# lusinlu/Video-Generation-for-Human-Avatars

Hardware: AMD Instinct MI355X
Metric: LTX-2B LoRA train-step samples/sec (latent-tokens/sec = samples/sec x 1792) (higher is better)
Workload: dtype bf16; 1 GPU; LTX-Video 2B LoRA(r=16, attn2 q/k/v/out) + caption_projection train step, 49f 512x512 -> latent 7x16x16 (N=1792), 1xMI355X per rank; lora_rank=16, model=LTX-Video-2B (28 layers, D 2048, 32x64 heads), global_batch=8, micro_batch_per_gpu=8, seq_len=1792, text_len=256, grad_accum=16, parallelism=dp1, attn2_padding_blocks=skipped, exact

## Files before the change

include/ltx_hip.h:

```cpp
#ifndef LTX_HIP_H_
#define LTX_HIP_H_

#include <stdint.h>

#ifdef __cplusplus
extern "C" {
#endif

enum {
  LTX_OK = 0,
  LTX_ERR_BAD_ARG = 1000,
  LTX_ERR_UNSUPPORTED = 1001,
};

enum {
  LTX_EPI_STORE = 0,
  LTX_EPI_GELU = 1,
  LTX_EPI_GATED_RESIDUAL = 2,
  LTX_EPI_LORA = 3,
  LTX_EPI_LORA_RESIDUAL = 4,
  LTX_EPI_GELU_BWD = 5,
  LTX_EPI_ACCUM = 6,
  LTX_EPI_LORA_DGRAD_ACCUM = 7,
  LTX_EPI_STORE_ROWDOT = 8,
// ... 132 lines not shown
                    int64_t ldo, void* stream);
int ltx_lora_rows(const void* x, int64_t ldx, const void* w3, int64_t ldw, float* out, int64_t ldo,
                  int64_t M, int64_t K, int64_t r, float alpha, void* split, int64_t ld_split,
                  int64_t K2, void* stream);
int ltx_lora_wgrad(const void* y, int64_t ldy, const float* u, int64_t ldu, float* dw,
                   int64_t on, int64_t oj, int64_t M, int64_t N, int64_t r, float alpha,
                   int accumulate, void* stream);
int ltx_lora_wgrad_grouped(const void* y, int64_t ldy, const float* u, int64_t ldu, float* dw,
                           int64_t on, int64_t oj, int64_t M, int64_t N, int64_t r, float alpha,
                           int accumulate, int64_t groups, int64_t gy, int64_t gu, int64_t gd,
                           void* stream);

int ltx_lora_dy(const void* y, int64_t ldy, const float* u, int64_t ldu, const void* w3, int64_t ldw3,
                int64_t M, int64_t N, int64_t r, float alpha, float* w, int64_t ldw_out, void* split,
                int64_t ld_split, int64_t K2, float* dw, int64_t on, int64_t oj, int accumulate,
                float* workspace, void* stream);
int ltx_lora_dy_workspace(int64_t M, int64_t N, int64_t r, int64_t* floats);
int ltx_lora_dy_dA(const void* y, int64_t ldy, const float* u, int64_t ldu, const void* w3, int64_t ldw3,
                   const void* x, int64_t ldx, int64_t M, int64_t N, int64_t K, int64_t r, float alpha,
                   float* w, int64_t ldw_out, void* split, int64_t ld_split, int64_t K2, float* dw,
                   int64_t on, int64_t oj, int accumulate, float alpha_a, float* dwa, int64_t ona,
                   int64_t oja, int acc_a, float* workspace, void* stream);
int ltx_lora_dy_dA_workspace(int64_t M, int64_t N, int64_t K, int64_t r, int64_t* floats);
int ltx_lora_rows_grouped(const void* x, int64_t ldx, const void* const* w3, int64_t ldw, float* out,
                          int64_t ldo, int64_t go, int64_t M, int64_t K, int64_t r, float alpha,
                          void* split, int64_t ld_split, int64_t K2, int64_t gs, int64_t groups,
                          void* stream);
int ltx_lora_dy_dA_grouped(const void* y, int64_t ldy, const float* const* u, int64_t ldu,
                           const void* const* w3, int64_t ldw3, const void* x, int64_t ldx, int64_t M,
                           int64_t N, int64_t K, int64_t r, int64_t groups, float alpha, float* w,
                           int64_t ldw_out, int64_t gw, void* split, int64_t ld_split, int64_t K2,
                           int64_t gs, float* const* dw, int64_t on, int64_t oj, int accumulate,
                           float alpha_a, float* const* dwa, int64_t ona, int64_t oja, int acc_a,
                           float* workspace, void* stream);
int ltx_lora_dy_dA_grouped_workspace(int64_t M, int64_t N, int64_t K, int64_t r, int64_t groups,
                                     int64_t* floats);

int ltx_lora_dropout_apply(const void* x, int64_t ldx, void* out, int64_t ldo, int64_t M, int64_t K,
                           uint64_t key, int64_t sid, int64_t T, void* stream);
int ltx_lora_up_masked_add(void* dx, int64_t lddx, const float* w, int64_t ldw, const float* const* A,
                           int64_t lda, const int64_t* sids, int64_t groups, int64_t M, int64_t K,
                           int64_t r, uint64_t key, int64_t T, float c, const void* gq, int64_t ldg,
                           void* stream);

int ltx_dora_fold(const void* W, int64_t ldw, const float* A, int64_t lda, const float* B, int64_t brs,
                  int64_t bcs, const float* m, float s, int64_t N, int64_t K, int64_t r, float* norm,
// ... 62 lines not shown
```

video-generation-for-human-avatars_amd/csrc/lora_dy.hip:

```cpp
#include <cstdlib>

#include "attention_common.h"
#include "ltx_hip.h"

namespace ltx {

#ifndef LTX_RF_NR
#define LTX_RF_NR 5
#endif
namespace {
constexpr int DY_NR = 4;
constexpr int DY_COLS = 512;
constexpr int DY_MAXCS = 4;
constexpr int dy_sw(int r) { return r <= 16 ? 16 : 32; }
constexpr int dy_g(int r) { return r <= 16 ? 7 : 4; }
constexpr int dy_nsl(int r) { return r <= 32 ? 1 : r / 32; }
constexpr bool dy_rank_ok(int64_t r) { return r == 8 || r == 16 || r == 32 || r == 64 || r == 128; }
}

template <int R, int MODE>
__global__ __launch_bounds__(512) void lora_dy_kernel(const bf16_t* __restrict__ y, int64_t ldy,
                                                      const float* __restrict__ u, int64_t ldu,
                                                      const bf16_t* __restrict__ w3, int64_t ldw,
                                                      float* __restrict__ part_w, float* __restrict__ part_b,
                                                      int M, int N, const float* __restrict__ part_u, int CSu,
                                                      float alpha_u) {
#define DY_BX blockIdx.x
#define DY_BY blockIdx.y
#define LTX_DY_BODY 1
#include "lora_dy_bodies.h"
#undef LTX_DY_BODY
#undef DY_BX
#undef DY_BY
}

constexpr int LORA_MAX_GROUPS = 4;
struct DyGroupPtrs {
  const float* u[LORA_MAX_GROUPS];
  const bf16_t* w3[LORA_MAX_GROUPS];
  float* dw[LORA_MAX_GROUPS];
  float* dwa[LORA_MAX_GROUPS];
};

template <int R, int MODE>
__global__ __launch_bounds__(512) void lora_dy_grouped_kernel(const bf16_t* __restrict__ y0, int64_t ldy,
                                                              DyGroupPtrs gp, int64_t ldu, int64_t ldw,
                                                              float* __restrict__ part_w0,
                                                              float* __restrict__ part_b0, int M, int N,
                                                              const float* __restrict__ part_u0, int CSu,
                                                              float alpha_u, int G, int64_t gy, int64_t gpw,
                                                              int64_t gpb, int64_t gpu) {
  unsigned g, gbx;
  if constexpr ((MODE & 4) != 0) {
// ... 61 lines not shown

template <int R>
__global__ __launch_bounds__(256) void lora_dy_finish_grouped_kernel(
    const float* __restrict__ part_w0, int CS, const float* __restrict__ part_b0, int RS, int M, int N, float alpha,
    float* __restrict__ w0, int64_t ldw_out, bf16_t* __restrict__ split0, int64_t lds, int K2, DyGroupPtrs gp,
    int64_t on, int64_t oj, int accumulate, int nwb, int nbb, const float* __restrict__ part_a0, int Na,
    float alpha_a, int64_t ona, int64_t oja, int acc_a, int64_t gpw, int64_t gpb, int64_t gpa, int64_t gwo,
    int64_t gso) {
  const unsigned g = blockIdx.y;
  const float* __restrict__ part_w = part_w0 + g * gpw;
  const float* __restrict__ part_b = part_b0 + g * gpb;
  const float* __restrict__ part_a = part_a0 + g * gpa;
  float* __restrict__ w = w0 + g * gwo;
  bf16_t* __restrict__ split = split0 + g * gso;
  float* __restrict__ dw = gp.dw[g];
  float* __restrict__ dwa = gp.dwa[g];
#define DY_BX blockIdx.x
#define DY_BY blockIdx.y
#define LTX_DY_BODY 2
#include "lora_dy_bodies.h"
#undef LTX_DY_BODY
#undef DY_BX
#undef DY_BY
}

template <int R, int RG, int CH, int NR>
__global__ __launch_bounds__(512) void lora_rows_full_kernel(const bf16_t* __restrict__ x, int64_t ldx,
                                                             const bf16_t* __restrict__ w3, int64_t ldw,
                                                             float* __restrict__ out, int64_t ldo, int M, float alpha,
                                                             bf16_t* __restrict__ split, int64_t lds, int K2) {
#define DY_BX blockIdx.x
#define DY_BY blockIdx.y
#define LTX_DY_BODY 3
#include "lora_dy_bodies.h"
#undef LTX_DY_BODY
#undef DY_BX
#undef DY_BY
}

struct RowsGroupPtrs {
  const bf16_t* w3[LORA_MAX_GROUPS];
};
template <int R, int RG, int CH, int NR>
__global__ __launch_bounds__(512) void lora_rows_full_grouped_kernel(const bf16_t* __restrict__ x, int64_t ldx,
                                                                     RowsGroupPtrs gp, int64_t ldw,
                                                                     float* __restrict__ out0, int64_t ldo, int M,
// ... 202 lines not shown
                     ldy, u, ldu, (const bf16_t*)w3, ldw3, pw, pb, (int)M, (int)N, (const float*)nullptr, 0, 1.f);  \
  LTX_LAUNCH_CHECK();                                                                                              \
  if (CS <= DY_MAXCS)                                                                                              \
    hipLaunchKernelGGL((lora_dy_kernel<RR, 6>), dim3((unsigned)(CSx * NSL), (unsigned)RS), dim3(512), 0, s,       \
                       (const bf16_t*)x, ldx, (const float*)nullptr, (int64_t)0, (const bf16_t*)nullptr,           \
                       (int64_t)0, (float*)nullptr, pa, (int)M, (int)K, (const float*)pw, CS, alpha);              \
  else                                                                                                             \
    hipLaunchKernelGGL((lora_dy_kernel<RR, 14>), dim3((unsigned)(CSx * NSL), (unsigned)RS), dim3(512), 0, s,      \
                       (const bf16_t*)x, ldx, (const float*)nullptr, (int64_t)0, (const bf16_t*)nullptr,           \
                       (int64_t)0, (float*)nullptr, pa, (int)M, (int)K, (const float*)pw, CS, alpha);              \
  LTX_LAUNCH_CHECK();                                                                                              \
  hipLaunchKernelGGL((lora_dy_finish_kernel<RR>), dim3((unsigned)(nwb + nbb + nba)), dim3(256), 0, s, pw, CS, pb,  \
                     RS, (int)M, (int)N, alpha, w, ldw_out, (bf16_t*)split, ld_split, (int)K2, dw, on, oj,         \
                     accumulate, nwb, nbb, (const float*)pa, (int)K, alpha_a, dwa, ona, oja, acc_a);
  switch (r) {
    case 8: LTX_LORA_DYA(8) break;
    case 16: LTX_LORA_DYA(16) break;
    case 32: LTX_LORA_DYA(32) break;
    case 64: LTX_LORA_DYA(64) break;
    case 128: LTX_LORA_DYA(128) break;
    default: return fail(LTX_ERR_BAD_ARG, "lora_dy_dA: rank must be 8, 16, 32, 64 or 128");
  }
#undef LTX_LORA_DYA
  LTX_LAUNCH_CHECK();
  return LTX_OK;
}

extern "C" int ltx_lora_dy_dA_grouped_workspace(int64_t M, int64_t N, int64_t K, int64_t r, int64_t groups,
                                                int64_t* floats) {
  LTX_CHECK_ARG(groups >= 1 && groups <= LORA_MAX_GROUPS, "lora_dy_dA_grouped_workspace: 1 to 4 groups");
  int64_t one = 0;
  const int rc = ltx_lora_dy_dA_workspace(M, N, K, r, &one);
  if (rc != LTX_OK) return rc;
  *floats = groups * one;
  return LTX_OK;
}

extern "C" int ltx_lora_dy_dA_grouped(const void* y, int64_t ldy, const float* const* u, int64_t ldu,
                                      const void* const* w3, int64_t ldw3, const void* x, int64_t ldx, int64_t M,
                                      int64_t N, int64_t K, int64_t r, int64_t groups, float alpha, float* w,
                                      int64_t ldw_out, int64_t gw, void* split, int64_t ld_split, int64_t K2,
                                      int64_t gs, float* const* dw, int64_t on, int64_t oj, int accumulate,
                                      float alpha_a, float* const* dwa, int64_t ona, int64_t oja, int acc_a,
                                      float* workspace, void* stream) {
  LTX_CHECK_ARG(y && u && w3 && x && w && split && dw && dwa && workspace, "lora_dy_dA_grouped: null operand");
  LTX_CHECK_ARG(groups >= 1 && groups <= LORA_MAX_GROUPS, "lora_dy_dA_grouped: 1 to 4 groups");
// ... 130 lines not shown
```

video-generation-for-human-avatars_amd/csrc/lora_dy_bodies.h:

```cpp
#if LTX_DY_BODY == 1
  constexpr int RP = R >= 16 ? R : 16;
  constexpr int SW = dy_sw(R);
  constexpr int NSL = dy_nsl(R);
  constexpr int DY_G = dy_g(R);
  constexpr int DY_UPAD = DY_G * 32 + 4;
  constexpr int JT = SW / 16;
  constexpr int NF = 3 * JT;
  constexpr int RING = 8 * DY_NR * 4096;
  constexpr int UT = SW * DY_UPAD * 4;
  static_assert(dy_rank_ok(R), "rank 8, 16, 32, 64 or 128");
  __shared__ __attribute__((aligned(16))) char smem[RING + UT];
  float* ut = (float*)(smem + RING);
  const int tid = threadIdx.x, lane = tid & 63;
  const int wave = __builtin_amdgcn_readfirstlane(tid >> 6);
  const int cs = DY_BX / NSL, rs = DY_BY;
  const int j0 = (DY_BX % NSL) * SW;
  const int c0 = cs * DY_COLS + wave * 64;
  const int mb = rs * DY_G * 32;

  uint32_t yo[4];
#pragma unroll
  for (int i = 0; i < 4; ++i) {
    const int row = 8 * i + (lane >> 3);
    yo[i] = (uint32_t)(row * ldy + (((lane & 7) ^ swz<64>(row)) * 8)) * 2;
// ... 81 lines not shown
#pragma unroll
      for (int c = 0; c < DY_MAXCS; ++c)
        if (c < CSu) acc += pv[i][c];
      uv[i] = (e < DY_G * 32 * SW && m < M && j < R) ? acc * alpha_u : 0.f;
    }
#pragma unroll
    for (int i = 0; i < UPT; ++i) {
      const int e = tid + 512 * i;
      if (e < DY_G * 32 * SW) ut[(e / (DY_G * 32)) * DY_UPAD + e % (DY_G * 32)] = uv[i];
    }
  } else {
#pragma unroll
    for (int i = 0; i < UPT; ++i) {
      const int e = tid + 512 * i, rr = e / SW, j = j0 + e % SW, m = mb + rr;
      uv[i] = ((MODE & 2) && e < DY_G * 32 * SW && m < M && j < R) ? u[(int64_t)m * ldu + j] : 0.f;
    }
#pragma unroll
    for (int i = 0; i < UPT; ++i) {
      const int e = tid + 512 * i;
      if ((MODE & 2) && e < DY_G * 32 * SW) ut[(e % SW) * DY_UPAD + e / SW] = uv[i];
    }
  }
  __syncthreads();

  int roff[2][2];
#pragma unroll
  for (int q = 0; q < 2; ++q)
#pragma unroll
    for (int h = 0; h < 2; ++h) {
      const int row = 16 * q + (lane & 15);
      roff[q][h] = row * 128 + (((4 * h + (lane >> 4)) ^ swz<64>(row)) * 16);
    }
  const int g4 = lane >> 4, qq = (lane & 15) >> 2, pp = lane & 3;
  int toffs[4];
#pragma unroll
  for (int nb = 0; nb < 4; ++nb) toffs[nb] = toff<64>(4 * g4 + qq, 2 * nb + (pp >> 1)) + 8 * (pp & 1);
  auto tr4 = [](const char* a) {
    return __builtin_amdgcn_ds_read_tr16_b64_v4i16((__attribute__((address_space(3))) s16x4*)a);
  };

  f32x4 wacc[DY_G][2][JT];
  f32x4 bacc[JT][4];
#pragma unroll
  for (int t = 0; t < JT; ++t)
#pragma unroll
    for (int nb = 0; nb < 4; ++nb) bacc[t][nb] = (f32x4){0.f, 0.f, 0.f, 0.f};
// ... 287 lines not shown
```

video-generation-for-human-avatars_amd/ltx_amd/_lib.py:

```python
import ctypes
import os
import threading

import torch

_HERE = os.path.dirname(os.path.abspath(__file__))
LIB_PATH = os.environ.get("LTX_HIP_LIB", os.path.join(_HERE, "libltxhip.so"))

_i64 = ctypes.c_int64
_i32 = ctypes.c_int
_f32 = ctypes.c_float
_p = ctypes.c_void_p

_SIGNATURES = {
    "ltx_abi_version": [],
    "ltx_device_info": [ctypes.POINTER(_i32), ctypes.POINTER(_i32)],
    "ltx_patchify_bf16": [_p, _p, _i64, _i64, _i64, _i64, _i64, _p],
    "ltx_unpatchify_bf16": [_p, _p, _i64, _i64, _i64, _i64, _i64, _p],
    "ltx_latent_coords": [_p, _i64, _i64, _i64, _i64, _p],
    "ltx_rf_noise_velocity": [_p, _p, _p, _p, _p, _i64, _i64, _p],
    "ltx_rf_noise_velocity_f32": [_p, _i32, _p, _i32, _p, _p, _p, _i64, _i64, _p],
    "ltx_condition_lerp": [_p, _p, _p, _p, _i64, _i64, _i64, _i64, _i64, _p],
    "ltx_rf_prepare_tokens": [_p, _p, _p, _p, _p, _p, _p, _p, _i64, _i64, _i64, _i64, _i64, _p],
    "ltx_rmsnorm_modulate_fwd": [_p, _p, _p, _i64, _p, _p, _i64, _i64, _i64, _f32, _p],
# ... 27 lines not shown
    "ltx_gemm_set_variant": [_i32],
    "ltx_gemm_describe": [_i64, _i64, _i64, _i64, _i32, _i64, _p, _p, _i64],
    "ltx_add_bf16": [_p, _i64, _p, _i64, _p, _i64, _i64, _i64, _p],
    "ltx_gated_residual_bf16": [_p, _i64, _p, _i64, _p, _i64, _p, _i64, _i64, _i64, _i64, _p],
    "ltx_gemm_set_workspace": [_p, _i64],
    "ltx_gemm_set_stream_workspace": [_p, _p, _i64],
    "ltx_gemm_bf16_nt_ext": [_p, _i64, _p, _i64, _p, _i64, _p, _i64, _i64, _p, _i64, _i64, _i64,
                             _i64, _i32, _p, _p, _i64, _p, _i64, _p, _i64, _f32, _i64, _i64, _p],
    "ltx_gemm_bf16_nt_gext": [_p, _i64, _p, _i64, _p, _i64, _p, _i64, _i64, _i64, _i64, _p, _i64,
                              _i64, _i64, _i64, _i32, _p, _p, _i64, _p, _i64, _p, _i64, _f32, _i64,
                              _i64, _p],
    "ltx_lora_down_grouped": [_p, _i64, _p, _i64, _i64, _p, _i64, _i64, _i64, _i64, _f32, _p, _i64,
                              _i64, _i64, _i64, _i64, _i64, _i64, _p],
    "ltx_lora_wgrad_grouped": [_p, _i64, _p, _i64, _p, _i64, _i64, _i64, _i64, _i64, _f32, _i32,
                               _i64, _i64, _i64, _i64, _p],
    "ltx_lora_pieces": [_p, _i64, _i64, _i64, _i64, _p, _i64, _p],
    "ltx_lora_rows": [_p, _i64, _p, _i64, _p, _i64, _i64, _i64, _i64, _f32, _p, _i64, _i64, _p],
    "ltx_lora_dy": [_p, _i64, _p, _i64, _p, _i64, _i64, _i64, _i64, _f32, _p, _i64, _p, _i64, _i64, _p,
                    _i64, _i64, _i32, _p, _p],
    "ltx_lora_dy_workspace": [_i64, _i64, _i64, ctypes.POINTER(_i64)],
    "ltx_lora_dy_dA": [_p, _i64, _p, _i64, _p, _i64, _p, _i64, _i64, _i64, _i64, _i64, _f32, _p, _i64,
                       _p, _i64, _i64, _p, _i64, _i64, _i32, _f32, _p, _i64, _i64, _i32, _p, _p],
    "ltx_lora_dy_dA_workspace": [_i64, _i64, _i64, _i64, ctypes.POINTER(_i64)],
    "ltx_lora_rows_grouped": [_p, _i64, ctypes.POINTER(_p), _i64, _p, _i64, _i64, _i64, _i64, _i64, _f32,
                              _p, _i64, _i64, _i64, _i64, _p],
    "ltx_lora_dy_dA_grouped": [_p, _i64, ctypes.POINTER(_p), _i64, ctypes.POINTER(_p), _i64, _p, _i64, _i64,
                               _i64, _i64, _i64, _i64, _f32, _p, _i64, _i64, _p, _i64, _i64, _i64,
                               ctypes.POINTER(_p), _i64, _i64, _i32, _f32, ctypes.POINTER(_p), _i64, _i64,
                               _i32, _p, _p],
    "ltx_lora_dy_dA_grouped_workspace": [_i64, _i64, _i64, _i64, _i64, ctypes.POINTER(_i64)],
    "ltx_lora_dropout_apply": [_p, _i64, _p, _i64, _i64, _i64, ctypes.c_uint64, _i64, _i64, _p],
    "ltx_lora_up_masked_add": [_p, _i64, _p, _i64, ctypes.POINTER(_p), _i64, ctypes.POINTER(_i64), _i64, _i64,
                               _i64, _i64, ctypes.c_uint64, _i64, _f32, _p, _i64, _p],
    "ltx_dora_fold": [_p, _i64, _p, _i64, _p, _i64, _i64, _p, _f32, _i64, _i64, _i64, _p, _p, _p, _i64, _p, _p],
    "ltx_dora_mag_grad": [_p, _i64, _p, _i64, _p, _p, _i64, _i64, _p, _i32, _p, _p],
    "ltx_dora_mag_grad_workspace": [_i64, _i64, ctypes.POINTER(_i64), ctypes.POINTER(_i64)],
    "ltx_dora_rowscale_add": [_p, _p, _f32, _i64, _i64, _p, _i64, _i64, _p],
    "ltx_lora_split_bf16": [_p, _i64, _i64, _f32, _i64, _i64, _i32, _p, _i64, _i64, _p],
    "ltx_lora_down": [_p, _i64, _p, _i64, _i64, _p, _i64, _i64, _i64, _i64, _f32, _p, _i64, _i64,
                      _p],
    "ltx_lora_wgrad": [_p, _i64, _p, _i64, _p, _i64, _i64, _i64, _i64, _i64, _f32, _i32, _p],
    "ltx_timestep_embedding": [_p, _f32, _p, _i64, _i64, _p],
    "ltx_silu_bf16": [_p, _p, _i64, _p],
    "ltx_transpose_bf16": [_p, _i64, _p, _i64, _i64, _i64, _p],
    "ltx_colsum_bf16": [_p, _i64, _p, _i64, _i64, _p],
    "ltx_batch_sum_bf16": [_p, _i64, _i64, _i64, _i64, _p, _i64, _p],
# ... 85 lines not shown
```

video-generation-for-human-avatars_amd/ltx_amd/ops.py:

```python
import ctypes
import functools
import os

import torch

from . import _lib
from ._lib import EPI, call

BF16 = torch.bfloat16
F32 = torch.float32


def _p(t):
    return None if t is None else ctypes.c_void_p(t.data_ptr())


def _s():
    return _lib.stream_ptr()


def _rows(t, name):
    if t.dim() != 2 or t.stride(1) != 1:
        raise ValueError(f"{name}: expected a 2-D row-major view, got shape {tuple(t.shape)} "
                         f"strides {t.stride()}")
# ... 709 lines not shown
    w = torch.empty(M, r, dtype=F32, device=y.device) if w_out is None else w_out
    sp = torch.empty(M, K2, dtype=BF16, device=y.device) if split_out is None else split_out
    assert w.shape == (M, r) and w.dtype == F32 and sp.shape == (M, K2) and sp.dtype == BF16
    n = ctypes.c_int64(0)
    if x is not None:
        K = x.shape[1]
        assert x.shape[0] == M and x.dtype == BF16 and lora_dy_fits(x, r) and N % 512 == 0
        assert tuple(dA_out.shape) == (r, K) and dA_out.dtype == F32 and dA_out.is_contiguous()
        call("ltx_lora_dy_dA_workspace", M, N, K, r, ctypes.byref(n))
        ws = torch.empty(n.value, dtype=F32, device=y.device)
        call("ltx_lora_dy_dA", _p(y), _rows(y, "y"), _p(u), _rows(u, "u"), _p(w3), _rows(w3, "w3"),
             _p(x), _rows(x, "x"), M, N, K, r, float(alpha), _p(w), _rows(w, "w"), _p(sp),
             _rows(sp, "split"), K2, _p(dB_out), on, oj, 1 if accumulate else 0, float(dA_alpha), _p(dA_out), 1,
             K, 1 if dA_accumulate else 0, _p(ws), _s())
        return w, sp
    call("ltx_lora_dy_workspace", M, N, r, ctypes.byref(n))
    ws = torch.empty(n.value, dtype=F32, device=y.device)
    call("ltx_lora_dy", _p(y), _rows(y, "y"), _p(u), _rows(u, "u"), _p(w3), _rows(w3, "w3"), M, N, r,
         float(alpha), _p(w), _rows(w, "w"), _p(sp), _rows(sp, "split"), K2, _p(dB_out), on, oj,
         1 if accumulate else 0, _p(ws), _s())
    return w, sp


@functools.lru_cache(maxsize=64)
def lora_dropout_threshold(p):
    p = float(p)
    if not 0.0 < p < 1.0:
        raise ValueError(f"LoRA dropout rate {p!r}: expected 0 < p < 1")
    T = min(max(int(round(p * 65536.0)), 1), 65535)
    c = float(torch.tensor(1.0, dtype=F32) / (torch.tensor(1.0, dtype=F32) - torch.tensor(T / 65536.0, dtype=F32)))
    return T, c


def lora_dropout_apply(x, key, sid, T, out=None):
    _need(x, BF16, "lora_dropout_apply x")
    M, K = x.shape
    out = torch.empty(M, K, dtype=BF16, device=x.device) if out is None else out
    timer = _timer
    label = "ltx::lora_dropout_apply_kernel"
    timer = timer if (timer is not None and timer.wants(label)) else None
    ev0 = timer.start() if timer is not None else None
    call("ltx_lora_dropout_apply", _p(x), _rows(x, "x"), _p(out), _rows(out, "out"), M, K,
         ctypes.c_uint64(int(key) & 0xFFFFFFFFFFFFFFFF), int(sid), int(T), _s())
    if timer is not None:
        timer.stop(label, 0.0, ev0, 4.0 * M * K)
    return out
# ... 297 lines not shown
```

video-generation-for-human-avatars_amd/ltx_amd/transformer3d.py:

```python
import glob
import json
import math
import os
from dataclasses import dataclass
from enum import Enum, auto
from pathlib import Path
from typing import Any, Dict, List, Optional

import torch
from torch import nn

from . import _lib, ops
from .patchifier import SymmetricPatchifier

OURS_TRANSFORMER_CONFIG = {
    "_class_name": "Transformer3DModel",
    "activation_fn": "gelu-approximate",
    "attention_bias": True,
    "attention_head_dim": 64,
    "attention_type": "default",
    "caption_channels": 4096,
    "cross_attention_dim": 2048,
    "double_self_attention": False,
    "dropout": 0.0,
# ... 557 lines not shown
        raise NotImplementedError("the attn1 adapters of one block must share rank and scaling")
    return lins


def _lora_params_ff(blk):
    net = blk._modules["ff"]._modules["net"]._modules
    lins = (net["0"]._modules["proj"], net["2"])
    kinds = [type(m) is LoraLinear for m in lins]
    if not all(kinds):
        if any(kinds):
            raise NotImplementedError("LoRA must wrap both feed-forward linears (ff.net.0.proj, ff.net.2) or none")
        return None
    if lins[0].r != lins[1].r or lins[0].scaling != lins[1].scaling:
        raise NotImplementedError("the feed-forward adapters of one block must share rank and scaling")
    return lins


def _ff_keep_x2():
    return os.environ.get("LTX_LORA_FF_KEEP_X2", "1") != "0"


def _ff_merge_da():
    return os.environ.get("LTX_LORA_FF_DY_DA", "0") == "1"


def _ab(m):
    return (m._modules["lora_A"]._modules["default"]._parameters["weight"],
            m._modules["lora_B"]._modules["default"]._parameters["weight"])


def _dora_m(m):
    return m._modules["lora_magnitude_vector"]._modules["default"]._parameters["weight"]


def _grad_buf(lin, which):
    p = _dora_m(lin) if which == "m" else _ab(lin)[0 if which == "A" else 1]
    if p.grad is None:
        p.grad = torch.zeros_like(p, memory_format=torch.contiguous_format)
    return p.grad


class _BlockFn(torch.autograd.Function):

    @staticmethod
    def forward(ctx, blk, sh, keep, skip, h, enc2, mods, onep, *lora_ab):
        B, N, L, H, d, D = sh.B, sh.N, sh.L, sh.H, sh.d, sh.D
# ... 149 lines not shown
            x1, y1, y3 = saved[24:27]
            dmods = torch.empty(B, 6, D, dtype=torch.bfloat16, device=h.device)
        if has_lora:
            Aq, Bq, Ak, Bk, Av, Bv, Ao, Bo = saved[24:32]
            u_q, u_k, u_v, u_o = saved[32:36]
            lora = _lora_params(blk)
            r, s = lora[0].r, lora[0].scaling
        dora = has_lora and lora[0].use_dora
        has1 = ctx.has1
        if has1:
            o1s = 36 if has_lora else 24
            ab1 = saved[o1s:o1s + 8]
            u1, u_o1, x1 = saved[o1s + 8:o1s + 11]
            lora1 = _lora_params1(blk)
            r1, s1 = lora1[0].r, lora1[0].scaling
        hasf = ctx.hasf
        if hasf:
            of = 24 + (12 if has_lora else 0) + (11 if has1 else 0)
            abf = saved[of:of + 4]
            u_f1, u_f2, act = saved[of + 4:of + 7]
            x2 = saved[of + 7] if len(saved) > of + 7 else None
            lf1, lf2 = _lora_params_ff(blk)
            rf, sf = lf1.r, lf1.scaling
        rpm = sh.rpm
        pre, sh.ffo_pre = sh.ffo_pre, None
        if pre is not None and pre[0].data_ptr() == dh3.data_ptr() and pre[0].shape == dh3.shape:
            d_ffo = pre[1]
        else:
            d_ffo = ops.gate_mul(dh3, mods[:, 5], rpm)
        del pre
        if full:
            ops.colsum_into(dmods[:, 5], dh3, y3, mode=1, rows_per_group=rpm, sum_groups=False,
                            accumulate=False)
        dp = ctx.dp
        ca = 1.0 if dp is None else dp[2]
        if hasf and dp is not None:
            xd = _drop_x(act, dp, 9)
            w2, _ = _lora_backward(d_ffo, u_f2, lf2, abf[3], xd, rf, sf, merge_da=_ff_merge_da(), da_alpha=ca)
            del xd
            d_f = ops.gemm(d_ffo, W["ff2_wT"], epilogue="gelu_bwd", aux0=fpre)
            _masked_add(d_f, w2, [abf[2]], dp, (9,), g=fpre)
            del d_ffo, act, w2
            if x2 is None:
                x2, _ = ops.rmsnorm_modulate_fwd(h2, mods[:, 3], onep[:, 4], ldm, rpm, blk.norm_eps)
            xd = _drop_x(x2, dp, 8)
            del x2
# ... 27 lines not shown
        del dx2
        fused2 = _DELTA_FUSED and not (has_lora and dp is not None)
        delta2 = torch.empty(B, H, N, dtype=torch.float32, device=h.device) if fused2 else None
        rd = dict(epilogue="store_rowdot", aux0=o2, aux1=delta2, rank=d, rows_per_batch=N) \
            if fused2 else {}
        if has_lora and dp is not None:
            lq, lk, lv, lo = lora
            xd = _drop_x(o2, dp, 7)
            w_o, _ = _lora_backward(dh2, u_o, lo, Bo, xd, r, s, da_alpha=ca)
            del xd
            do2 = ops.gemm(dh2, W["o2_wT"])
            _masked_add(do2, w_o, [Ao], dp, (7,))
            del w_o
        elif dora:
            lq, lk, lv, lo = lora
            _, sw = _lora_backward(dh2, u_o, lo, None, o2, r, s, dora=True)
            do2 = ops.gemm(dh2, W["o2_wT"], ext=(sw, lo.weight_split("A")), **rd)
            yo = ops.gemm(o2, W["o2_w"], ext=(ops.lora_split(u_o, "act"), lo.weight_split("B")))
            ops.dora_mag_grad(dh2, yo, None, _dora_m(lo), _grad_buf(lo, "m"))
            del yo
        elif has_lora:
            lq, lk, lv, lo = lora
            dy_ok = ops.lora_dy_enabled() and ops.lora_dy_fits(dh2, r)
            if dy_ok and ops.lora_dy_da_fits(dh2, o2, r):
                w_o, sw = ops.lora_dy(dh2, u_o, lo.weight_pieces("Bt"), r, s, _grad_buf(lo, "B"),
                                      x=o2, dA_out=_grad_buf(lo, "A"))
            else:
                if dy_ok:
                    w_o, sw = ops.lora_dy(dh2, u_o, lo.weight_pieces("Bt"), r, s, _grad_buf(lo, "B"))
                else:
                    ops.lora_wgrad(dh2, u_o, alpha=s, out=_grad_buf(lo, "B"), accumulate=True)
                    w_o, sw = ops.lora_down(dh2, Bo, alpha=s, transposed=True, split=True,
                                             pieces=lambda: lo.weight_pieces("Bt"))
                ops.lora_wgrad(o2, w_o, transpose_out=True, out=_grad_buf(lo, "A"), accumulate=True)
            do2 = ops.gemm(dh2, W["o2_wT"], ext=(sw, lo.weight_split("A")), **rd)
        else:
            do2 = ops.gemm(dh2, W["o2_wT"], **rd)
        if full:
            lin = a2.to_out[0]
            ops.wgrad_into(_pgrad(lin.weight), dh2, o2)
            ops.colsum_into(_pgrad(lin.bias), dh2)
        tx = sh.text_stack
        if tx is not None:
            dkv = tx.block_dkv(blk)
        else:
            dkv = torch.empty(k2raw.shape[0], 2 * D, dtype=torch.bfloat16, device=h.device)
        dk2b = dv2b = None
# ... 21 lines not shown
        else:
            dk2raw = None
        if full:
            ops.qk_norm_wgrad_into(dq2, q2raw, rq2, _pgrad(a2.q_norm.weight), B=B, N=N)
            ops.wgrad_into(_pgrad(a2.to_q.weight), dq2raw, h1)
            ops.colsum_into(_pgrad(a2.to_q.bias), dq2raw)
            if dk2b is not None:
                krep, erep, rrep = k2raw.repeat(B, 1), enc2.repeat(B, 1), rk2.repeat(B)
                dk2raw_b, _ = ops.qk_norm_rope_bwd(dk2b, krep, a2.k_norm.weight, rrep, B=B, N=L)
                ops.qk_norm_wgrad_into(dk2b, krep, rrep, _pgrad(a2.k_norm.weight), B=B, N=L)
                ops.wgrad_into(_pgrad(a2.to_k.weight), dk2raw_b, erep)
                ops.colsum_into(_pgrad(a2.to_k.bias), dk2raw_b)
                ops.wgrad_into(_pgrad(a2.to_v.weight), dv2b, erep)
                ops.colsum_into(_pgrad(a2.to_v.bias), dv2b)
                del krep, erep, rrep, dk2raw_b, dk2b, dv2b
            else:
                ops.qk_norm_wgrad_into(dk2, k2raw, rk2, _pgrad(a2.k_norm.weight), B=sh.Bt, N=L)
                ops.wgrad_into(_pgrad(a2.to_k.weight), dk2raw, enc2)
                ops.colsum_into(_pgrad(a2.to_k.bias), dk2raw)
                ops.wgrad_into(_pgrad(a2.to_v.weight), dv2, enc2)
                ops.colsum_into(_pgrad(a2.to_v.bias), dv2)
        del dq2, dk2
        denc = None
        d_y1 = torch.empty_like(dh2)
        gated = dict(aux1=mods[:, 2], aux2=d_y1, rows_per_batch=rpm)
        if has_lora and dp is not None:
            xd = _drop_x(h1, dp, 4)
            w_q, _ = _lora_backward(dq2raw, u_q, lq, Bq, xd, r, s, da_alpha=ca)
            del xd
            dh1 = ops.gemm(dq2raw, W["q2_wT"], epilogue="accum", aux0=dh2)
            _masked_add(dh1, w_q, [Aq], dp, (4,))
            del w_q
            d_y1 = ops.gate_mul(dh1, mods[:, 2], rpm)
            w_kv = torch.empty(dkv.shape[0], 2 * r, dtype=torch.float32, device=h.device)
            for i, (dy, u_t, lt, Bt_) in enumerate(((dk2raw, u_k, lk, Bk), (dv2, u_v, lv, Bv))):
                ops.lora_wgrad(dy, u_t, alpha=s, out=_grad_buf(lt, "B"), accumulate=True)
                ops.lora_down(dy, Bt_, alpha=s, transposed=True, out=w_kv[:, i * r:(i + 1) * r])
                xd = _drop_x(enc2, dp, 5 + i)
                ops.lora_wgrad(xd, w_kv[:, i * r:(i + 1) * r], alpha=ca, transpose_out=True,
                               out=_grad_buf(lt, "A"), accumulate=True)
                del xd
            denc = ops.gemm(dkv, W["kv2_wT"])
            _masked_add(denc, w_kv, [Ak, Av], dp, (5, 6))
            del w_kv
            grads_lora = grads_lora + [None] * 8
        elif dora:
            _, sw = _lora_backward(dq2raw, u_q, lq, None, h1, r, s, dora=True)
            dh1 = ops.gemm(dq2raw, W["q2_wT"], epilogue="accum", aux0=dh2,
                           ext=(sw, lq.weight_split("A")), **gated)
            ops.dora_mag_grad(dq2raw, q2raw, _lin(lq)[1], _dora_m(lq), _grad_buf(lq, "m"))
            K2 = ops.lora_k2(r)
            swkv = torch.empty(dkv.shape[0], 2 * K2, dtype=torch.bfloat16, device=h.device)
            for i, (dy, y_t, u_t, lt) in enumerate(((dk2raw, k2raw, u_k, lk), (dv2, v2, u_v, lv))):
                dop = lt.dora_operands()
                dB = ops.lora_wgrad(dy, u_t)
                ops.dora_rowscale_add(_grad_buf(lt, "B"), dB, dop["c"], s)
                w_t, _ = ops.lora_down(dy, dop["sB"], transposed=True, split=True,
                                       split_out=swkv[:, i * K2:(i + 1) * K2])
                ops.lora_wgrad(enc2, w_t, transpose_out=True, out=_grad_buf(lt, "A"), accumulate=True)
                ops.dora_mag_grad(dy, y_t, _lin(lt)[1], _dora_m(lt), _grad_buf(lt, "m"))
            denc = ops.gemm(dkv, W["kv2_wT"], ext=(swkv, _kv_ext(blk, lk, lv)[1]))
            del swkv
            grads_lora = grads_lora + [None] * 8
        elif has_lora:
            dy_ok = ops.lora_dy_enabled() and ops.lora_dy_fits(dq2raw, r)
            if dy_ok and ops.lora_dy_da_fits(dq2raw, h1, r):
                w_q, sw = ops.lora_dy(dq2raw, u_q, lq.weight_pieces("Bt"), r, s, _grad_buf(lq, "B"),
                                      x=h1, dA_out=_grad_buf(lq, "A"))
            else:
                if dy_ok:
                    w_q, sw = ops.lora_dy(dq2raw, u_q, lq.weight_pieces("Bt"), r, s, _grad_buf(lq, "B"))
                else:
                    ops.lora_wgrad(dq2raw, u_q, alpha=s, out=_grad_buf(lq, "B"), accumulate=True)
                    w_q, sw = ops.lora_down(dq2raw, Bq, alpha=s, transposed=True, split=True,
                                             pieces=lambda: lq.weight_pieces("Bt"))
                ops.lora_wgrad(h1, w_q, transpose_out=True, out=_grad_buf(lq, "A"), accumulate=True)
            dh1 = ops.gemm(dq2raw, W["q2_wT"], epilogue="accum", aux0=dh2,
                           ext=(sw, lq.weight_split("A")), **gated)
            if tx is None:
                K2 = ops.lora_k2(r)
                swkv = torch.empty(dkv.shape[0], 2 * K2, dtype=torch.bfloat16, device=h.device)
                ops.lora_wgrad(dk2raw, u_k, alpha=s, out=_grad_buf(lk, "B"), accumulate=True)
                w_k, _ = ops.lora_down(dk2raw, Bk, alpha=s, transposed=True, split=True,
                                       split_out=swkv[:, :K2])
                ops.lora_wgrad(enc2, w_k, transpose_out=True, out=_grad_buf(lk, "A"),
                               accumulate=True)
                ops.lora_wgrad(dv2, u_v, alpha=s, out=_grad_buf(lv, "B"), accumulate=True)
                w_v, _ = ops.lora_down(dv2, Bv, alpha=s, transposed=True, split=True,
                                       split_out=swkv[:, K2:])
                ops.lora_wgrad(enc2, w_v, transpose_out=True, out=_grad_buf(lv, "A"),
                               accumulate=True)
                denc = ops.gemm(dkv, W["kv2_wT"], ext=(swkv, _kv_ext(blk, lk, lv)[1]))
                del swkv
            grads_lora = grads_lora + [None] * 8
        else:
            dh1 = ops.gemm(dq2raw, W["q2_wT"], epilogue="accum", aux0=dh2, **gated)
            if tx is None:
                denc = ops.gemm(dkv, W["kv2_wT"])
        del dq2raw, dk2raw, dv2, dh2, dkv
        fused1 = _DELTA_FUSED and not (has1 and dp is not None)
        delta1 = torch.empty(B, H, N, dtype=torch.float32, device=h.device) if fused1 else None
        rd = dict(epilogue="store_rowdot", aux0=o1, aux1=delta1, rank=d, rows_per_batch=N) \
            if fused1 else {}
        if has1 and dp is not None:
            lo1 = lora1[3]
            xd = _drop_x(o1, dp, 3)
            w_o1, _ = _lora_backward(d_y1, u_o1, lo1, ab1[7], xd, r1, s1, da_alpha=ca)
            del xd
            do1 = ops.gemm(d_y1, W["out1_wT"])
            _masked_add(do1, w_o1, [ab1[6]], dp, (3,))
            del w_o1
            grads_lora = grads_lora + [None] * 8
        elif has1:
            lo1 = lora1[3]
            _, sw = _lora_backward(d_y1, u_o1, lo1, ab1[7], o1, r1, s1)
            do1 = ops.gemm(d_y1, W["out1_wT"], ext=(sw, lo1.weight_split("A")), **rd)
            del sw
            grads_lora = grads_lora + [None] * 8
        else:
            do1 = ops.gemm(d_y1, W["out1_wT"], **rd)
        if full:
            ops.colsum_into(dmods[:, 2], dh1, y1, mode=1, rows_per_group=rpm, sum_groups=False,
# ... 767 lines not shown
```

Measured before the change: 68.50 samples/s.

## Split LoRA dY/dA into pass kernels with merged reduce; prune unneeded backward branch

Measured after the change: 68.96 samples/s (median of 6 runs). About the same (+0.7%).

```diff
diff --git a/include/ltx_hip.h b/include/ltx_hip.h
--- a/include/ltx_hip.h
+++ b/include/ltx_hip.h
@@ -178,6 +178,16 @@
                    int64_t on, int64_t oj, int accumulate, float alpha_a, float* dwa, int64_t ona,
                    int64_t oja, int acc_a, float* workspace, void* stream);
 int ltx_lora_dy_dA_workspace(int64_t M, int64_t N, int64_t K, int64_t r, int64_t* floats);
+int ltx_lora_dy_dA_passes(const void* y, int64_t ldy, const float* u, int64_t ldu, const void* w3,
+                          int64_t ldw3, const void* x, int64_t ldx, int64_t M, int64_t N, int64_t K,
+                          int64_t r, float alpha, float* w, int64_t ldw_out, void* split,
+                          int64_t ld_split, int64_t K2, float* workspace, void* stream);
+int ltx_lora_dy_dA_partials(int64_t M, int64_t N, int64_t K, int64_t r, int64_t* off_b, int64_t* off_a,
+                            int64_t* floats);
+int ltx_lora_dy_reduce(int64_t count, const float* const* part, const int64_t* part_floats,
+                       const int64_t* M, const int64_t* N, const float* alpha, float* const* out,
+                       const int64_t* on, const int64_t* oj, const int* accumulate, int64_t r,
+                       void* stream);
 int ltx_lora_rows_grouped(const void* x, int64_t ldx, const void* const* w3, int64_t ldw, float* out,
                           int64_t ldo, int64_t go, int64_t M, int64_t K, int64_t r, float alpha,
                           void* split, int64_t ld_split, int64_t K2, int64_t gs, int64_t groups,
diff --git a/video-generation-for-human-avatars_amd/csrc/lora_dy.hip b/video-generation-for-human-avatars_amd/csrc/lora_dy.hip
--- a/video-generation-for-human-avatars_amd/csrc/lora_dy.hip
+++ b/video-generation-for-human-avatars_amd/csrc/lora_dy.hip
@@ -29,6 +29,28 @@
 #define DY_BY blockIdx.y
 #define LTX_DY_BODY 1
 #include "lora_dy_bodies.h"
+#undef LTX_DY_BODY
+#undef DY_BX
+#undef DY_BY
+}
+
+template <int R, int MODE>
+__global__ __launch_bounds__(512) void lora_dy_xw_kernel(const bf16_t* __restrict__ y, int64_t ldy,
+                                                         float* __restrict__ part_b, int M, int N,
+                                                         const float* __restrict__ part_u, int CSu, float alpha_u,
+                                                         float* __restrict__ w_out, int64_t ldw_out,
+                                                         bf16_t* __restrict__ split, int64_t lds, int K2) {
+  static_assert((MODE & 7) == 6, "the x pass: dA from the dY pass's w partials");
+  constexpr const float* u = nullptr;
+  constexpr const bf16_t* w3 = nullptr;
+  constexpr float* part_w = nullptr;
+  constexpr int64_t ldu = 0, ldw = 0;
+#define DY_BX blockIdx.x
+#define DY_BY blockIdx.y
+#define LTX_DY_BODY 1
+#define LTX_DY_WOUT 1
+#include "lora_dy_bodies.h"
+#undef LTX_DY_WOUT
 #undef LTX_DY_BODY
 #undef DY_BX
 #undef DY_BY
@@ -136,6 +158,39 @@
 #undef LTX_DY_BODY
 #undef DY_BX
 #undef DY_BY
+}
+
+struct DyReduceArgs {
+  const float* part[LORA_MAX_GROUPS];
+  float* out[LORA_MAX_GROUPS];
+  int64_t on[LORA_MAX_GROUPS], oj[LORA_MAX_GROUPS];
+  float alpha[LORA_MAX_GROUPS];
+  int rs[LORA_MAX_GROUPS], n[LORA_MAX_GROUPS], acc[LORA_MAX_GROUPS];
+  int blk0[LORA_MAX_GROUPS];
+};
+template <int R>
+__global__ __launch_bounds__(256) void lora_dy_reduce_kernel(DyReduceArgs a) {
+  __shared__ float red[4][64];
+  const int b = (int)blockIdx.x;
+  const float* part = a.part[0];
+  float* out = a.out[0];
+  int64_t on = a.on[0], oj = a.oj[0];
+  float alpha = a.alpha[0];
+  int rs = a.rs[0], n = a.n[0], acc = a.acc[0], b0 = 0;
+#pragma unroll
+  for (int t = 1; t < LORA_MAX_GROUPS; ++t)
+    if (b >= a.blk0[t]) {
+      part = a.part[t];
+      out = a.out[t];
+      on = a.on[t];
+      oj = a.oj[t];
+      alpha = a.alpha[t];
+      rs = a.rs[t];
+      n = a.n[t];
+      acc = a.acc[t];
+      b0 = a.blk0[t];
+    }
+  finish_rows<R>(part, rs, n, alpha, out, on, oj, acc, b - b0, red);
 }
 
 template <int R, int RG, int CH, int NR>
@@ -384,6 +439,109 @@
     default: return fail(LTX_ERR_BAD_ARG, "lora_dy_dA: rank must be 8, 16, 32, 64 or 128");
   }
 #undef LTX_LORA_DYA
+  LTX_LAUNCH_CHECK();
+  return LTX_OK;
+}
+
+extern "C" int ltx_lora_dy_dA_partials(int64_t M, int64_t N, int64_t K, int64_t r, int64_t* off_b, int64_t* off_a,
+                                       int64_t* floats) {
+  LTX_CHECK_ARG(off_b && off_a && floats, "lora_dy_dA_partials: null output");
+  const int rc = ltx_lora_dy_dA_workspace(M, N, K, r, floats);
+  if (rc != LTX_OK) return rc;
+  const int64_t RP = r >= 16 ? r : 16;
+  const int64_t DY_G = dy_g((int)r);
+  const int64_t CS = N / DY_COLS, RS = (M + DY_G * 32 - 1) / (DY_G * 32);
+  *off_b = CS * M * RP;
+  *off_a = *off_b + RS * N * RP;
+  return LTX_OK;
+}
+
+extern "C" int ltx_lora_dy_dA_passes(const void* y, int64_t ldy, const float* u, int64_t ldu, const void* w3,
+                                     int64_t ldw3, const void* x, int64_t ldx, int64_t M, int64_t N, int64_t K,
+                                     int64_t r, float alpha, float* w, int64_t ldw_out, void* split,
+                                     int64_t ld_split, int64_t K2, float* workspace, void* stream) {
+  LTX_CHECK_ARG(y && u && w3 && x && w && workspace, "lora_dy_dA_passes: null operand");
+  LTX_CHECK_ARG(r == 8 || r == 16, "lora_dy_dA_passes: rank 8 or 16");
+  LTX_CHECK_ARG(M >= 32 && M % 32 == 0 && N >= DY_COLS && N % DY_COLS == 0 && K >= DY_COLS && K % DY_COLS == 0,
+                "lora_dy_dA_passes: M % 32 == 0, N % 512 == 0, K % 512 == 0");
+  LTX_CHECK_ARG(ldy % 8 == 0 && ((uintptr_t)y % 16) == 0 && ldy >= N && ldw3 % 8 == 0 && ((uintptr_t)w3 % 16) == 0 &&
+                    ldw3 >= N,
+                "lora_dy_dA_passes: 16-B aligned rows of dY and of the pieces");
+  LTX_CHECK_ARG(ldx % 8 == 0 && ((uintptr_t)x % 16) == 0 && ldx >= K, "lora_dy_dA_passes: 16-B aligned rows of x");
+  LTX_CHECK_ARG(ldy * 2 * 32 < ((int64_t)1 << 32) && ldx * 2 * 32 < ((int64_t)1 << 32),
+                "lora_dy_dA_passes: 32-bit DMA offsets");
+  LTX_CHECK_ARG(M * (r >= 16 ? r : 16) * (N / DY_COLS) < ((int64_t)1 << 31), "lora_dy_dA_passes: partials too large");
+  LTX_CHECK_ARG(ldw_out >= r && ldu >= r && ldw_out % 4 == 0 && ((uintptr_t)w % 16) == 0,
+                "lora_dy_dA_passes: 16-B aligned w rows");
+  LTX_CHECK_ARG(!split || (K2 >= 3 * r && K2 % 64 == 0 && ld_split >= K2 && ld_split % 4 == 0 &&
+                           ((uintptr_t)split % 8) == 0),
+                "lora_dy_dA_passes: 8-B aligned split rows of K2 >= 3r, K2 % 64 == 0 columns");
+  const int64_t RP = r >= 16 ? r : 16;
+  const int DY_G = dy_g((int)r);
+  const int CS = (int)(N / DY_COLS), CSx = (int)(K / DY_COLS), RS = (int)((M + DY_G * 32 - 1) / (DY_G * 32));
+  float* pw = workspace;
+  float* pb = pw + (int64_t)CS * M * RP;
+  float* pa = pb + (int64_t)RS * N * RP;
+  hipStream_t s = (hipStream_t)stream;
+#define LTX_LORA_DYP(RR)                                                                                           \
+  hipLaunchKernelGGL((lora_dy_kernel<RR, 3>), dim3((unsigned)CS, (unsigned)RS), dim3(512), 0, s, (const bf16_t*)y, \
+                     ldy, u, ldu, (const bf16_t*)w3, ldw3, pw, pb, (int)M, (int)N, (const float*)nullptr, 0, 1.f);  \
+  LTX_LAUNCH_CHECK();                                                                                              \
+  if (CS <= DY_MAXCS)                                                                                              \
+    hipLaunchKernelGGL((lora_dy_xw_kernel<RR, 6>), dim3((unsigned)CSx, (unsigned)RS), dim3(512), 0, s,            \
+                       (const bf16_t*)x, ldx, pa, (int)M, (int)K, (const float*)pw, CS, alpha, w, ldw_out,         \
+                       (bf16_t*)split, ld_split, (int)K2);                                                         \
+  else                                                                                                             \
+    hipLaunchKernelGGL((lora_dy_xw_kernel<RR, 14>), dim3((unsigned)CSx, (unsigned)RS), dim3(512), 0, s,           \
+                       (const bf16_t*)x, ldx, pa, (int)M, (int)K, (const float*)pw, CS, alpha, w, ldw_out,         \
+                       (bf16_t*)split, ld_split, (int)K2);
+  if (r == 8) {
+    LTX_LORA_DYP(8)
+  } else {
+    LTX_LORA_DYP(16)
+  }
+#undef LTX_LORA_DYP
+  LTX_LAUNCH_CHECK();
+  return LTX_OK;
+}
+
+extern "C" int ltx_lora_dy_reduce(int64_t count, const float* const* part, const int64_t* part_floats,
+                                  const int64_t* M, const int64_t* N, const float* alpha, float* const* out,
+                                  const int64_t* on, const int64_t* oj, const int* accumulate, int64_t r,
+                                  void* stream) {
+  LTX_CHECK_ARG(count >= 1 && count <= LORA_MAX_GROUPS, "lora_dy_reduce: 1 to 4 tuples");
+  LTX_CHECK_ARG(part && part_floats && M && N && alpha && out && on && oj && accumulate && (r == 8 || r == 16),
+                "lora_dy_reduce: null argument or bad rank (8 or 16, the ranks of ltx_lora_dy_dA_passes)");
+  const int64_t RP = r >= 16 ? r : 16;
+  const int64_t DY_G = dy_g((int)r);
+  DyReduceArgs a{};
+  int64_t blocks = 0;
+  for (int t = 0; t < (int)count; ++t) {
+    LTX_CHECK_ARG(part[t] && out[t] && M[t] > 0 && N[t] > 0, "lora_dy_reduce: null or empty tuple");
+    LTX_CHECK_ARG((on[t] == r && oj[t] == 1) || (on[t] == 1 && oj[t] == N[t]),
+                  "lora_dy_reduce: every output a dense [N,r] or [r,N]");
+    const int64_t RS = (M[t] + DY_G * 32 - 1) / (DY_G * 32);
+    LTX_CHECK_ARG(RS * N[t] * RP <= part_floats[t], "lora_dy_reduce: partials smaller than the row splits need");
+    LTX_CHECK_ARG(N[t] * r < ((int64_t)1 << 31) && RS < ((int64_t)1 << 31), "lora_dy_reduce: sizes");
+    a.part[t] = part[t];
+    a.out[t] = out[t];
+    a.on[t] = on[t];
+    a.oj[t] = oj[t];
+    a.alpha[t] = alpha[t];
+    a.rs[t] = (int)RS;
+    a.n[t] = (int)N[t];
+    a.acc[t] = accumulate[t];
+    a.blk0[t] = (int)blocks;
+    blocks += (N[t] * r + 63) / 64;
+    LTX_CHECK_ARG(blocks < ((int64_t)1 << 31), "lora_dy_reduce: too many blocks");
+  }
+  for (int t = (int)count; t < LORA_MAX_GROUPS; ++t) a.blk0[t] = 0x7fffffff;
+  hipStream_t s = (hipStream_t)stream;
+#define LTX_LORA_RED(RR) \
+  hipLaunchKernelGGL((lora_dy_reduce_kernel<RR>), dim3((unsigned)blocks), dim3(256), 0, s, a)
+  if (r == 8) LTX_LORA_RED(8);
+  else LTX_LORA_RED(16);
+#undef LTX_LORA_RED
   LTX_LAUNCH_CHECK();
   return LTX_OK;
 }
diff --git a/video-generation-for-human-avatars_amd/csrc/lora_dy_bodies.h b/video-generation-for-human-avatars_amd/csrc/lora_dy_bodies.h
--- a/video-generation-for-human-avatars_amd/csrc/lora_dy_bodies.h
+++ b/video-generation-for-human-avatars_amd/csrc/lora_dy_bodies.h
@@ -127,6 +127,34 @@
     }
   }
   __syncthreads();
+#ifdef LTX_DY_WOUT
+  {
+    constexpr int NQ = (R < SW ? R : SW) / 4;
+    const int nsp = N / DY_COLS, rows = (DY_G * 32 + nsp - 1) / nsp;
+    for (int t = tid; t < rows * NQ; t += 512) {
+      const int q = t % NQ, rr = cs * rows + t / NQ, m = mb + rr;
+      if (rr >= DY_G * 32 || m >= M) continue;
+      f32x4 wv;
+#pragma unroll
+      for (int k = 0; k < 4; ++k) wv[k] = ut[(4 * q + k) * DY_UPAD + rr];
+      const int jq = j0 + 4 * q;
+      *(f32x4*)(w_out + (int64_t)m * ldw_out + jq) = wv;
+      if (split == nullptr) continue;
+      uint32_t hi[2], lo[2];
+#pragma unroll
+      for (int k = 0; k < 2; ++k) {
+        const bf16_t h0 = f2bf(wv[2 * k]), h1 = f2bf(wv[2 * k + 1]);
+        hi[k] = (uint32_t)h0 | ((uint32_t)h1 << 16);
+        lo[k] = (uint32_t)f2bf(wv[2 * k] - bf2f(h0)) | ((uint32_t)f2bf(wv[2 * k + 1] - bf2f(h1)) << 16);
+      }
+      bf16_t* sr = split + (int64_t)m * lds;
+      *(u32x2*)(sr + jq) = (u32x2){hi[0], hi[1]};
+      *(u32x2*)(sr + R + jq) = (u32x2){hi[0], hi[1]};
+      *(u32x2*)(sr + 2 * R + jq) = (u32x2){lo[0], lo[1]};
+      for (int cc = 3 * R + jq; cc < K2; cc += R) *(u32x2*)(sr + cc) = (u32x2){0u, 0u};
+    }
+  }
+#endif
 
   int roff[2][2];
 #pragma unroll
diff --git a/video-generation-for-human-avatars_amd/ltx_amd/_lib.py b/video-generation-for-human-avatars_amd/ltx_amd/_lib.py
--- a/video-generation-for-human-avatars_amd/ltx_amd/_lib.py
+++ b/video-generation-for-human-avatars_amd/ltx_amd/_lib.py
@@ -73,6 +73,13 @@
     "ltx_lora_dy_dA": [_p, _i64, _p, _i64, _p, _i64, _p, _i64, _i64, _i64, _i64, _i64, _f32, _p, _i64,
                        _p, _i64, _i64, _p, _i64, _i64, _i32, _f32, _p, _i64, _i64, _i32, _p, _p],
     "ltx_lora_dy_dA_workspace": [_i64, _i64, _i64, _i64, ctypes.POINTER(_i64)],
+    "ltx_lora_dy_dA_passes": [_p, _i64, _p, _i64, _p, _i64, _p, _i64, _i64, _i64, _i64, _i64, _f32, _p, _i64,
+                              _p, _i64, _i64, _p, _p],
+    "ltx_lora_dy_dA_partials": [_i64, _i64, _i64, _i64, ctypes.POINTER(_i64), ctypes.POINTER(_i64),
+                                ctypes.POINTER(_i64)],
+    "ltx_lora_dy_reduce": [_i64, ctypes.POINTER(_p), ctypes.POINTER(_i64), ctypes.POINTER(_i64),
+                           ctypes.POINTER(_i64), ctypes.POINTER(_f32), ctypes.POINTER(_p), ctypes.POINTER(_i64),
+                           ctypes.POINTER(_i64), ctypes.POINTER(_i32), _i64, _p],
     "ltx_lora_rows_grouped": [_p, _i64, ctypes.POINTER(_p), _i64, _p, _i64, _i64, _i64, _i64, _i64, _f32,
                               _p, _i64, _i64, _i64, _i64, _p],
     "ltx_lora_dy_dA_grouped": [_p, _i64, ctypes.POINTER(_p), _i64, ctypes.POINTER(_p), _i64, _p, _i64, _i64,
diff --git a/video-generation-for-human-avatars_amd/ltx_amd/ops.py b/video-generation-for-human-avatars_amd/ltx_amd/ops.py
--- a/video-generation-for-human-avatars_amd/ltx_amd/ops.py
+++ b/video-generation-for-human-avatars_amd/ltx_amd/ops.py
@@ -755,6 +755,53 @@
     return w, sp
 
 
+_LORA_FINISH_MERGED = os.environ.get("LTX_LORA_FINISH_MERGED", "1") != "0"
+
+
+def lora_finish_merged_fits(y, x, r):
+    return _LORA_FINISH_MERGED and r in (8, 16) and lora_dy_da_fits(y, x, r)
+
+
+def lora_dy_passes(y, u, w3, r, alpha, dB_out, x, dA_out, accumulate=True, dA_accumulate=True, w_out=None,
+                   split_out=None, want_split=True, dA_alpha=1.0):
+    M, N = y.shape
+    K = x.shape[1]
+    assert tuple(dB_out.shape) == (N, r) and dB_out.dtype == F32 and dB_out.is_contiguous()
+    assert tuple(dA_out.shape) == (r, K) and dA_out.dtype == F32 and dA_out.is_contiguous()
+    assert x.shape[0] == M and x.dtype == BF16 and y.dtype == BF16 and lora_dy_fits(x, r) and lora_dy_fits(y, r)
+    K2 = lora_k2(r)
+    w = torch.empty(M, r, dtype=F32, device=y.device) if w_out is None else w_out
+    assert w.shape == (M, r) and w.dtype == F32
+    sp = None
+    if want_split:
+        sp = torch.empty(M, K2, dtype=BF16, device=y.device) if split_out is None else split_out
+        assert sp.shape == (M, K2) and sp.dtype == BF16
+    ob, oa, n = ctypes.c_int64(0), ctypes.c_int64(0), ctypes.c_int64(0)
+    call("ltx_lora_dy_dA_partials", M, N, K, r, ctypes.byref(ob), ctypes.byref(oa), ctypes.byref(n))
+    ws = torch.empty(n.value, dtype=F32, device=y.device)
+    call("ltx_lora_dy_dA_passes", _p(y), _rows(y, "y"), _p(u), _rows(u, "u"), _p(w3), _rows(w3, "w3"),
+         _p(x), _rows(x, "x"), M, N, K, r, float(alpha), _p(w), _rows(w, "w"), _p(sp),
+         _rows(sp, "split") if sp is not None else 0, K2 if sp is not None else 0, _p(ws), _s())
+    pending = [(ws[ob.value:oa.value], M, N, float(alpha), dB_out, r, 1, bool(accumulate)),
+               (ws[oa.value:n.value], M, K, float(dA_alpha), dA_out, 1, K, bool(dA_accumulate))]
+    return w, sp, pending
+
+
+LORA_REDUCE_MAX = 4
+
+
+def lora_dy_reduce(pending, r):
+    for i in range(0, len(pending), LORA_REDUCE_MAX):
+        grp = pending[i:i + LORA_REDUCE_MAX]
+        c = len(grp)
+        call("ltx_lora_dy_reduce", c, _ptr_array([g[0] for g in grp]),
+             (ctypes.c_int64 * c)(*[g[0].numel() for g in grp]), (ctypes.c_int64 * c)(*[g[1] for g in grp]),
+             (ctypes.c_int64 * c)(*[g[2] for g in grp]), (ctypes.c_float * c)(*[g[3] for g in grp]),
+             _ptr_array([g[4] for g in grp]), (ctypes.c_int64 * c)(*[g[5] for g in grp]),
+             (ctypes.c_int64 * c)(*[g[6] for g in grp]), (ctypes.c_int * c)(*[1 if g[7] else 0 for g in grp]),
+             r, _s())
+
+
 @functools.lru_cache(maxsize=64)
 def lora_dropout_threshold(p):
     p = float(p)
diff --git a/video-generation-for-human-avatars_amd/ltx_amd/transformer3d.py b/video-generation-for-human-avatars_amd/ltx_amd/transformer3d.py
--- a/video-generation-for-human-avatars_amd/ltx_amd/transformer3d.py
+++ b/video-generation-for-human-avatars_amd/ltx_amd/transformer3d.py
@@ -603,6 +603,9 @@
 
 def _ff_merge_da():
     return os.environ.get("LTX_LORA_FF_DY_DA", "0") == "1"
+
+
+_BWD_PRUNE = os.environ.get("LTX_BWD_PRUNE", "1") != "0"
 
 
 def _ab(m):
@@ -798,6 +801,8 @@
             x2 = saved[of + 7] if len(saved) > of + 7 else None
             lf1, lf2 = _lora_params_ff(blk)
             rf, sf = lf1.r, lf1.scaling
+        need1 = not _BWD_PRUNE or ctx.needs_input_grad[4] or full or has1
+        red2 = []
         rpm = sh.rpm
         pre, sh.ffo_pre = sh.ffo_pre, None
         if pre is not None and pre[0].data_ptr() == dh3.data_ptr() and pre[0].shape == dh3.shape:
@@ -871,7 +876,10 @@
         elif has_lora:
             lq, lk, lv, lo = lora
             dy_ok = ops.lora_dy_enabled() and ops.lora_dy_fits(dh2, r)
-            if dy_ok and ops.lora_dy_da_fits(dh2, o2, r):
+            if dy_ok and ops.lora_finish_merged_fits(dh2, o2, r):
+                w_o, sw, red2 = ops.lora_dy_passes(dh2, u_o, lo.weight_pieces("Bt"), r, s, _grad_buf(lo, "B"),
+                                                   o2, _grad_buf(lo, "A"))
+            elif dy_ok and ops.lora_dy_da_fits(dh2, o2, r):
                 w_o, sw = ops.lora_dy(dh2, u_o, lo.weight_pieces("Bt"), r, s, _grad_buf(lo, "B"),
                                       x=o2, dA_out=_grad_buf(lo, "A"))
             else:
@@ -939,16 +947,18 @@
                 ops.colsum_into(_pgrad(a2.to_v.bias), dv2)
         del dq2, dk2
         denc = None
-        d_y1 = torch.empty_like(dh2)
+        dh1 = None
+        d_y1 = torch.empty_like(dh2) if need1 else None
         gated = dict(aux1=mods[:, 2], aux2=d_y1, rows_per_batch=rpm)
         if has_lora and dp is not None:
             xd = _drop_x(h1, dp, 4)
             w_q, _ = _lora_backward(dq2raw, u_q, lq, Bq, xd, r, s, da_alpha=ca)
             del xd
-            dh1 = ops.gemm(dq2raw, W["q2_wT"], epilogue="accum", aux0=dh2)
-            _masked_add(dh1, w_q, [Aq], dp, (4,))
+            if need1:
+                dh1 = ops.gemm(dq2raw, W["q2_wT"], epilogue="accum", aux0=dh2)
+                _masked_add(dh1, w_q, [Aq], dp, (4,))
+                d_y1 = ops.gate_mul(dh1, mods[:, 2], rpm)
             del w_q
-            d_y1 = ops.gate_mul(dh1, mods[:, 2], rpm)
             w_kv = torch.empty(dkv.shape[0], 2 * r, dtype=torch.float32, device=h.device)
             for i, (dy, u_t, lt, Bt_) in enumerate(((dk2raw, u_k, lk, Bk), (dv2, u_v, lv, Bv))):
                 ops.lora_wgrad(dy, u_t, alpha=s, out=_grad_buf(lt, "B"), accumulate=True)
@@ -963,8 +973,9 @@
             grads_lora = grads_lora + [None] * 8
         elif dora:
             _, sw = _lora_backward(dq2raw, u_q, lq, None, h1, r, s, dora=True)
-            dh1 = ops.gemm(dq2raw, W["q2_wT"], epilogue="accum", aux0=dh2,
-                           ext=(sw, lq.weight_split("A")), **gated)
+            if need1:
+                dh1 = ops.gemm(dq2raw, W["q2_wT"], epilogue="accum", aux0=dh2,
+                               ext=(sw, lq.weight_split("A")), **gated)
             ops.dora_mag_grad(dq2raw, q2raw, _lin(lq)[1], _dora_m(lq), _grad_buf(lq, "m"))
             K2 = ops.lora_k2(r)
             swkv = torch.empty(dkv.shape[0], 2 * K2, dtype=torch.bfloat16, device=h.device)
@@ -981,7 +992,13 @@
             grads_lora = grads_lora + [None] * 8
         elif has_lora:
             dy_ok = ops.lora_dy_enabled() and ops.lora_dy_fits(dq2raw, r)
-            if dy_ok and ops.lora_dy_da_fits(dq2raw, h1, r):
+            if dy_ok and ops.lora_finish_merged_fits(dq2raw, h1, r):
+                w_q, sw, red_q = ops.lora_dy_passes(dq2raw, u_q, lq.weight_pieces("Bt"), r, s,
+                                                    _grad_buf(lq, "B"), h1, _grad_buf(lq, "A"),
+                                                    want_split=need1)
+                red2 = red2 + red_q
+                del red_q
+            elif dy_ok and ops.lora_dy_da_fits(dq2raw, h1, r):
                 w_q, sw = ops.lora_dy(dq2raw, u_q, lq.weight_pieces("Bt"), r, s, _grad_buf(lq, "B"),
                                       x=h1, dA_out=_grad_buf(lq, "A"))
             else:
@@ -992,8 +1009,12 @@
                     w_q, sw = ops.lora_down(dq2raw, Bq, alpha=s, transposed=True, split=True,
                                              pieces=lambda: lq.weight_pieces("Bt"))
                 ops.lora_wgrad(h1, w_q, transpose_out=True, out=_grad_buf(lq, "A"), accumulate=True)
-            dh1 = ops.gemm(dq2raw, W["q2_wT"], epilogue="accum", aux0=dh2,
-                           ext=(sw, lq.weight_split("A")), **gated)
+            if red2:
+                ops.lora_dy_reduce(red2, r)
+                red2 = []
+            if need1:
+                dh1 = ops.gemm(dq2raw, W["q2_wT"], epilogue="accum", aux0=dh2,
+                               ext=(sw, lq.weight_split("A")), **gated)
             if tx is None:
                 K2 = ops.lora_k2(r)
                 swkv = torch.empty(dkv.shape[0], 2 * K2, dtype=torch.bfloat16, device=h.device)
@@ -1011,10 +1032,16 @@
                 del swkv
             grads_lora = grads_lora + [None] * 8
         else:
-            dh1 = ops.gemm(dq2raw, W["q2_wT"], epilogue="accum", aux0=dh2, **gated)
+            if need1:
+                dh1 = ops.gemm(dq2raw, W["q2_wT"], epilogue="accum", aux0=dh2, **gated)
             if tx is None:
                 denc = ops.gemm(dkv, W["kv2_wT"])
         del dq2raw, dk2raw, dv2, dh2, dkv
+        if not need1:
+            done = None if tx is None else tx.token_params[tx.index[id(blk)]]
+            for cb in getattr(blk, "_grad_ready_hooks", ()):
+                cb(blk, done)
+            return (None, None, None, None, None, denc, None, None, *grads_lora)
         fused1 = _DELTA_FUSED and not (has1 and dp is not None)
         delta1 = torch.empty(B, H, N, dtype=torch.float32, device=h.device) if fused1 else None
         rd = dict(epilogue="store_rowdot", aux0=o1, aux1=delta1, rank=d, rows_per_batch=N) \
```
